# LiHaoy-ux/DQO-MAP

Measured on AMD Instinct MI355X. Metric: mapping iters/sec (fwd+bwd raster) @ 500k Gaussians 1200×680; PSNR vs ref, higher is better.
Workload: dtype f32; 1 GPU; cfg3: surfel room, ONE map of 500000 Gaussians, 1200x680, 8 object ids, SH degree 3, per-object render (object gate) + per-object masked loss (sum over objects of 0.8 L1 colour + 1.0 depth L1 on the object's own mask) + attach loss, raster fwd+bwd + Adam (6 groups); path=fused (hipGraph replays of 4 iterations each); rccl_ranks=1, backend=none (one rank), list_split=0, list_split_backward=0, graph_unroll=4, sync_mode=lazy, selfcheck=skipped, P=500000, P_visible=196562, view=room, adam=exact-sparse, adam_rows_touched=148371, attach_loss_members=49997

## Files before the change

### dqo-map_amd/csrc/dqo_capi.hip

```cpp
#include <stdarg.h>
#include <stdio.h>
#include <string.h>

#include "dqo_common.h"

static thread_local char g_err[512] = "";

void dqo_set_error(const char* fmt, ...) {
    va_list ap;
    va_start(ap, fmt);
    vsnprintf(g_err, sizeof(g_err), fmt, ap);
    va_end(ap);
}

#include <map>
#include <mutex>
#include <string>
#include <vector>
int g_dqo_profile_on = 0;
namespace {
std::mutex g_profile_mu;
struct Pending {
    std::string name;
    hipEvent_t start, stop;
// ... 65 lines not shown
                                sizeof(DqoAdamTensor), sizeof(DqoRastParamInputs), sizeof(DqoRastParamGrads), 0 ,
                                sizeof(DqoLifecycle), sizeof(DqoGrowthSample)};
    return (which >= 0 && which < (int32_t)(sizeof(sz) / sizeof(sz[0]))) ? sz[which] : 0;
}
DQO_API const char* dqo_last_error(void) { return g_err; }

DQO_API size_t dqo_rast_geom_bytes(int32_t P, int32_t W, int32_t H) {
    (void)W;
    (void)H;
    return dqo_geom_layout(nullptr, P < 0 ? 0 : P).total;
}
DQO_API size_t dqo_rast_image_bytes(int32_t W, int32_t H) { return dqo_image_layout(nullptr, W, H).total; }
DQO_API size_t dqo_rast_binning_bytes(int64_t cap) { return dqo_bin_layout(nullptr, cap < 0 ? 0 : cap, cap < 0 ? 0 : cap, 0).total; }
DQO_API size_t dqo_rast_binning_bytes_bucketed(int64_t cap, int32_t W, int32_t H, int32_t bucket) {
    if (cap < 0) cap = 0;
    if (bucket <= 0 || W <= 0 || H <= 0) return dqo_rast_binning_bytes(cap);
    return dqo_bin_layout(nullptr, cap, dqo_list_cap(cap, W, H, bucket), bucket).total;
}
DQO_API size_t dqo_rast_backward_workspace_bytes(int64_t cap) { return dqo_bwd_ws_bytes(cap); }

static int check_common(const DqoRastParams* p, const DqoRastInputs* in, const DqoRastCtx* ctx) {
    DQO_CHECK_ARG(p && in && ctx, "null params / inputs / ctx");
    DQO_CHECK_ARG(p->P >= 0 && p->W > 0 && p->H > 0, "bad sizes P=%d W=%d H=%d", p->P, p->W, p->H);
    DQO_CHECK_ARG(p->D >= 0 && p->D <= 3, "sh degree %d out of range 0..3", p->D);
    DQO_CHECK_ARG((p->W + DQO_TILE - 1) / DQO_TILE < 65536 && (p->H + DQO_TILE - 1) / DQO_TILE < 65536, "image too large");
    DQO_CHECK_ARG(in->viewmatrix && in->projmatrix && in->campos && in->bg, "viewmatrix/projmatrix/campos/bg must be given");
    if (p->P > 0) {
        DQO_CHECK_ARG(in->means3D && in->opacities, "means3D / opacities missing");
        DQO_CHECK_ARG((in->shs != nullptr) != (in->colors_precomp != nullptr),
                      "Please provide excatly one of either SHs or precomputed colors!");
        DQO_CHECK_ARG(in->cov3D_precomp == nullptr,
                      "cov3D_precomp is not supported by the depth rasteriser: its blend kernel reads scales/rotations (forward.cu:780)");
        DQO_CHECK_ARG(in->scales && in->rotations, "scales and rotations are required");
        if (in->shs) DQO_CHECK_ARG(p->M >= (p->D + 1) * (p->D + 1), "sh has %d coefficients, degree %d needs %d", p->M, p->D, (p->D + 1) * (p->D + 1));
        if (in->colors_precomp == nullptr && p->M == 0) {
            dqo_set_error("For non-RGB, provide precomputed Gaussian colors!");
            return DQO_ERR_INVALID_ARG;
        }
    }
    DQO_CHECK_ARG(ctx->geom && ctx->geom_bytes >= dqo_rast_geom_bytes(p->P, p->W, p->H), "geom buffer too small (%zu < %zu)",
                  ctx->geom_bytes, dqo_rast_geom_bytes(p->P, p->W, p->H));
    DQO_CHECK_ARG(ctx->image && ctx->image_bytes >= dqo_rast_image_bytes(p->W, p->H), "image buffer too small (%zu < %zu)",
                  ctx->image_bytes, dqo_rast_image_bytes(p->W, p->H));
    return DQO_OK;
}

// ... 221 lines not shown
```

### dqo-map_amd/csrc/dqo_common.h

```cpp
#pragma once
#include <hip/hip_runtime.h>
#include <stdint.h>

#include "../../include/dqo_raster.h"
#include "dqo_activate.h"

#define DQO_TILE 16
#define DQO_WAVE 64
#define DQO_SPREAD 64
#define DQO_GATE_OBJECTS 64
#define DQO_OBJ_SPREAD 16
#ifndef DQO_TSTRIDE
#define DQO_TSTRIDE 64
#endif

#define DQO_API __attribute__((visibility("default")))

void dqo_set_error(const char* fmt, ...);
#define DQO_CHECK_ARG(cond, ...)          \
    do {                                  \
        if (!(cond)) {                    \
            dqo_set_error(__VA_ARGS__);   \
            return DQO_ERR_INVALID_ARG;   \
        }                                 \
// ... 194 lines not shown
    }
#pragma unroll
    for (int off = 32; off > 0; off >>= 1)
#pragma unroll
        for (int c = 0; c < 4; c++) t[c] += (unsigned long long)__shfl_xor((long long)t[c], off);
    tot[0] = (double)t[0] / DQO_TAP_FIXED, tot[1] = (double)t[1], tot[2] = (double)t[2] / DQO_TAP_FIXED, tot[3] = (double)t[3];
}
__device__ __forceinline__ unsigned long long dqo_tap_fixed(float s) {
    return (s >= 0.f && s < 2147483648.f) ? (unsigned long long)((double)s * DQO_TAP_FIXED + 0.5) : ~0ull >> 1;
}
#endif

static inline int dqo_list_split(const DqoRastCtx* ctx) { return ctx->list_split <= 0 ? 0 : (ctx->list_split < 64 ? 64 : ctx->list_split); }
struct DqoImageLayout {
    uint32_t* tile_count;
    uint32_t* tile_flag;
    uint32_t* tile_cursor;
    uint2* ranges;
    uint32_t* walk4;
    uint32_t* tile_order;
    uint4* slot_info;
    float* final_T;
    uint32_t* n_contrib;
    uint32_t* hit_pos;
    uint32_t* long_tiles;
    uint32_t* split_tiles;
    size_t total;
};

static inline DqoImageLayout dqo_image_layout(void* base, int W, int H) {
    DqoImageLayout L;
    const size_t gx = (W + DQO_TILE - 1) / DQO_TILE, gy = (H + DQO_TILE - 1) / DQO_TILE;
    const size_t T = gx * gy, HW = (size_t)W * H;
    char* p = (char*)base;
    auto take = [&](size_t bytes) {
        char* r = p;
        p += dqo_align_up(bytes, 256);
        return r;
    };
    L.tile_count = (uint32_t*)take(4 * T * DQO_TSTRIDE);
    L.tile_flag = (uint32_t*)take(4 * T);
    L.tile_cursor = (uint32_t*)take(4 * T * DQO_TSTRIDE);
    L.ranges = (uint2*)take(8 * T);
    L.walk4 = (uint32_t*)take(16 * T);
    L.tile_order = (uint32_t*)take(4 * 8 * ((T + 7) / 8));
    L.slot_info = (uint4*)take(16 * 8 * ((T + 7) / 8));
    L.final_T = (float*)take(4 * HW);
    L.n_contrib = (uint32_t*)take(4 * HW);
    L.hit_pos = (uint32_t*)take(4 * HW);
    L.long_tiles = (uint32_t*)take(4 * T);
    L.split_tiles = (uint32_t*)take(4 * T);
    L.total = (size_t)(p - (char*)base);
    return L;
}

struct DqoBinLayout {
    uint4* recs;
    uint32_t* point_list;
    uint32_t* slot_list;
    uint8_t* live_q;
    uint2* slot_info;
    uint32_t* slot_gid;
    uint32_t* rec_valid;
    int64_t list_cap;
    int32_t bucket;
    size_t total;
};
static inline int64_t dqo_list_cap(int64_t cap, int W, int H, int bucket) {
    const int64_t T = (int64_t)((W + DQO_TILE - 1) / DQO_TILE) * ((H + DQO_TILE - 1) / DQO_TILE);
    return bucket > 0 ? T * bucket : cap;
}

static inline DqoBinLayout dqo_bin_layout(void* base, int64_t cap, int64_t list_cap, int bucket) {
    DqoBinLayout L;
    L.list_cap = list_cap, L.bucket = bucket;
    char* p = (char*)base;
    auto take = [&](size_t bytes) {
        char* r = p;
// ... 175 lines not shown
```

### dqo-map_amd/csrc/rast_backward_blend.hip

```cpp
#include <type_traits>

#include "dqo_common.h"
#include "dqo_cull.h"

namespace {

template <int CTRL, int ROW_MASK = 0xF>
__device__ __forceinline__ float dpp_mov(float v) {
    return __int_as_float(__builtin_amdgcn_update_dpp(0, __float_as_int(v), CTRL, ROW_MASK, 0xF, false));
}
__device__ __forceinline__ float wave_sum(float v) {
    v += dpp_mov<0xB1>(v);
    v += dpp_mov<0x4E>(v);
    v += dpp_mov<0x141>(v);
    v += dpp_mov<0x140>(v);
    v += dpp_mov<0x142, 0xA>(v);
    v += dpp_mov<0x143, 0xC>(v);
    return __int_as_float(__builtin_amdgcn_readlane(__float_as_int(v), 63));
}

__device__ __forceinline__ uint32_t row0_sum_u32(uint32_t v) {
    v += (uint32_t)__builtin_amdgcn_update_dpp(0, (int)v, 0xB1, 0xF, 0xF, false);
    v += (uint32_t)__builtin_amdgcn_update_dpp(0, (int)v, 0x4E, 0xF, 0xF, false);
    v += (uint32_t)__builtin_amdgcn_update_dpp(0, (int)v, 0x141, 0xF, 0xF, false);
// ... 165 lines not shown
        tap.loss_out[4] = r4, tap.loss_out[5] = r5, tap.loss_out[6] = r6, tap.loss_out[7] = r7;
    }
}

constexpr int BWD_THREADS = 64;
constexpr int BWD_BLK = 3 * BWD_THREADS * 4 + 3 * BWD_THREADS + 5 * BWD_THREADS;
constexpr int BWD_XCH = 5 * BWD_THREADS;

#ifndef DQO_BWD_RG
#define DQO_BWD_RG 42
#endif
constexpr int RG = DQO_BWD_RG;
constexpr int RNB = 7;
constexpr int RNV = 64;
constexpr int RLS = 8;
static_assert(RG % RNB == 0 && RG >= RNB && (RG / RNB) * RLS <= 64 && (RG / RNB) * RLS - 2 < 63, "RG: whole batches, 64 list slots per row, slot 63 free");
constexpr int R_ENT_W = 12;
constexpr int R_ENT = 0;
constexpr int R_LIST = R_ENT + (RG + 1) * R_ENT_W;
constexpr int R_NB = RG / RNB;
constexpr int R_PART = R_LIST + 4 * 64 / 2;
constexpr int R_PART_W = 4 * R_NB * RNV + 12;
constexpr int R_MPOS = R_PART + R_PART_W;
constexpr int R_MCODE = R_MPOS + 64;
constexpr int ROWS_BLK = ((R_MCODE + 16 + 3) / 4) * 4;
static_assert(R_LIST % 4 == 0 && R_PART % 4 == 0, "16-byte aligned tables");
static_assert(5 * 64 <= R_PART_W, "the depth-hit staging fits the partial table");

struct BwdTap {
    float gc, gdw;
};
__device__ __forceinline__ BwdTap tap_frame_scales(const DqoGeomLayout& g, const DqoTapDev& tap, int lane, bool report) {
    BwdTap t;
    if (!report) {
        uint32_t c1, c3;
        dqo_tap_counts(g.spread, lane, c1, c3);
        const float n_col = fmaxf((float)c1, 1.f), n_dep = fmaxf((float)c3, 1.f);
        t.gc = tap.color_weight / (3.f * n_col), t.gdw = tap.depth_weight / n_dep;
        return t;
    }
    double tot[4];
    dqo_tap_totals(g.spread, lane, tot);
    const float n_col = fmaxf((float)tot[1], 1.f), n_dep = fmaxf((float)tot[3], 1.f);
    t.gc = tap.color_weight / (3.f * n_col), t.gdw = tap.depth_weight / n_dep;
    if (report && lane == 0) {
        const float color_loss = (float)(tot[0] / (3.0 * (double)n_col)), depth_loss = (float)(tot[2] / (double)n_dep);
        tap.loss_out[0] = tap.depth_weight * depth_loss + tap.color_weight * color_loss;
        tap.loss_out[1] = color_loss, tap.loss_out[2] = depth_loss, tap.loss_out[3] = 0.f;
        tap.loss_out[4] = (float)tot[0], tap.loss_out[5] = (float)tot[1], tap.loss_out[6] = (float)tot[2], tap.loss_out[7] = (float)tot[3];
        tap.scale[0] = t.gc, tap.scale[1] = t.gdw;
// ... 8 lines not shown
                                                   const DqoTapDev& tap, const DqoGateDev& gate, const int tile, const int quad, const int wave, const int lane, uint32_t* const lds, const int skip_over,
                                                   const uint2 range) {
    constexpr bool ROWS = SEGS == 1;
    uint32_t* const blk = lds + wave * (ROWS ? ROWS_BLK : BWD_BLK);
    float4* const s_co = reinterpret_cast<float4*>(blk);
    float4* const s_xy = s_co + BWD_THREADS;
    float4* const s_rgb = s_xy + BWD_THREADS;
    int* const s_id = reinterpret_cast<int*>(s_rgb + BWD_THREADS);
    uint32_t* const s_slot = reinterpret_cast<uint32_t*>(s_id + BWD_THREADS);
    int* const s_pos = reinterpret_cast<int*>(s_slot + BWD_THREADS);
    float* const s_hit = ROWS ? reinterpret_cast<float*>(blk + R_PART) : reinterpret_cast<float*>(s_pos + BWD_THREADS);
    const int n = (int)(range.y - range.x);
    if (n == 0 || n > skip_over) return;
    const int L = min((int)img.walk4[tile * 4 + quad], n);
    if (L == 0) return;
    const int tile_x = tile % v.gx, tile_y = tile / v.gx;
    const size_t HW = (size_t)v.W * v.H;
    const uint32_t px = tile_x * DQO_TILE + (quad & 1) * 8 + dqo_lane_x(lane);
    const uint32_t py = tile_y * DQO_TILE + (quad >> 1) * 8 + dqo_lane_y(lane);
    const bool inside = px < (uint32_t)v.W && py < (uint32_t)v.H;
    const size_t pid = (size_t)v.W * py + px;
    const float pixfx = (float)px, pixfy = (float)py;
    const uint8_t* const live = bin.live_q + (size_t)quad * (size_t)bin.list_cap + range.x;
    const size_t ps = inside ? pid : (size_t)0;
    const float T_final_ld = img.final_T[ps];
    const uint32_t n_contrib_ld = img.n_contrib[ps], hit_word_ld = img.hit_pos[ps];
    int owner_ld = 0;
    if (GATE) owner_ld = gate.pobj[ps];
    float in0, in1, in2, in3, in4 = 0.f, in5 = 0.f, in6 = 0.f, in7 = 0.f;
    uint8_t mask_ld = 1;
    if (tap.scale == nullptr) {
        in0 = dL_dpixels[ps], in1 = dL_dpixels[HW + ps], in2 = dL_dpixels[2 * HW + ps], in3 = dL_ddepths[ps];
    } else {
        if (tap.mask) mask_ld = tap.mask[ps];
        in0 = tap.out_color[ps], in1 = tap.out_color[HW + ps], in2 = tap.out_color[2 * HW + ps], in3 = tap.out_depth[ps];
        in4 = tap.gt_color[ps], in5 = tap.gt_color[HW + ps], in6 = tap.gt_color[2 * HW + ps], in7 = tap.gt_depth[ps];
    }
    uint8_t lv_first = 0;
    if (ROWS) lv_first = (L - 1 - lane >= 0) ? live[L - 1 - lane] : (uint8_t)0;
    float tap_gc = 0.f, tap_gdw = 0.f;
    if (tap.scale != nullptr && !(GATE && tap.per_object)) {
        const BwdTap t = tap_frame_scales(g, tap, lane, false);
        tap_gc = t.gc, tap_gdw = t.gdw;
    }
    const float T_final = inside ? T_final_ld : 0.f;
    float T = T_final;
    const int last_contrib = inside ? (int)n_contrib_ld : 0;
    const uint32_t hit_word = inside ? hit_word_ld : 0u;
    const int hit_pos = (int)(hit_word & 0x7fffffffu);
    const bool hit_plane = (hit_word >> 31) != 0u;
    const int hit_c0 = hit_pos - 1;
    const bool has_hit = hit_pos > 0;
    const int gid_h = (int)bin.point_list[range.x + max(hit_c0, 0)];
    const uint32_t slot_h_ld = bin.slot_list[range.x + max(hit_c0, 0)];
    char* const ent_base = reinterpret_cast<char*>(blk + R_ENT);
    int* const s_mpos = reinterpret_cast<int*>(blk + R_MPOS);
    uint8_t* const s_mcode = reinterpret_cast<uint8_t*>(blk + R_MCODE);
    const int chunks = (L + BWD_THREADS - 1) / BWD_THREADS;
    int chunk_i = 0;
    unsigned long long pend = 0ull;
    uint32_t my_code = 0u;
    uint8_t lv_nx = lv_first;
    auto below = [](unsigned long long m) { return (int)__builtin_amdgcn_mbcnt_hi((uint32_t)(m >> 32), __builtin_amdgcn_mbcnt_lo((uint32_t)m, 0u)); };
    int cnt = 0;
    auto collect = [&]() -> int {
        int cnt = 0;
        while (cnt < RG) {
            if (pend == 0ull) {
                if (chunk_i >= chunks) break;
                my_code = (uint32_t)lv_nx & 0xfu;
                chunk_i++;
                const int pn = L - 1 - (chunk_i * BWD_THREADS + lane);
                lv_nx = pn >= 0 ? live[pn] : (uint8_t)0;
                pend = __builtin_amdgcn_ballot_w64(my_code != 0u);
                continue;
            }
            const int rank = below(pend);
            const bool take = ((pend >> lane) & 1ull) != 0ull && rank < RG - cnt;
            if (take) s_mpos[cnt + rank] = L - 1 - ((chunk_i - 1) * BWD_THREADS + lane), s_mcode[cnt + rank] = (uint8_t)my_code;
            const unsigned long long tm = __builtin_amdgcn_ballot_w64(take);
            cnt += (int)__popcll(tm);
            pend &= ~tm;
        }
        return cnt;
    };
    int g_id = 0;
    auto gather_ids = [&](const int c) { g_id = (int)bin.point_list[range.x + (lane < c ? s_mpos[lane] : 0)]; };
    if constexpr (ROWS) {
        cnt = collect();
        gather_ids(cnt);
    }
    int owner = (int)0x80000000;
    if (GATE) {
        if (inside) owner = owner_ld;
        if (owner < 0) owner = (int)0x80000000;
        if (tap.scale != nullptr && tap.per_object) {
            unsigned long long todo = __builtin_amdgcn_ballot_w64(owner >= 0);
            while (todo != 0ull) {
                const int f = (int)__builtin_ctzll(todo);
                const int o = __builtin_amdgcn_readlane(owner, f);
                const unsigned long long* l = g.obj_tap + ((size_t)(lane & (DQO_OBJ_SPREAD - 1)) * DQO_GATE_OBJECTS + (size_t)(o & (DQO_GATE_OBJECTS - 1))) * 4;
                static_assert(DQO_OBJ_SPREAD <= 16, "the copies sit in one DPP row");
                const uint32_t n1 = row0_sum_u32(lane < DQO_OBJ_SPREAD ? (uint32_t)l[1] : 0u);
                const uint32_t n3 = row0_sum_u32(lane < DQO_OBJ_SPREAD ? (uint32_t)l[3] : 0u);
                const float n_col = fmaxf((float)n1, 1.f), n_dep = fmaxf((float)n3, 1.f);
                const bool mine = owner == o;
                tap_gc = mine ? tap.color_weight / (3.f * n_col) : tap_gc;
                tap_gdw = mine ? tap.depth_weight / n_dep : tap_gdw;
                todo &= ~__builtin_amdgcn_ballot_w64(mine);
            }
        }
    }
    float dp0 = 0.f, dp1 = 0.f, dp2 = 0.f, ddep = 0.f;
// ... 4 lines not shown
        const bool m = mask_ld != 0 && (!(GATE && tap.per_object) || owner >= 0);
        const float d0 = in0 - in4, d1 = in1 - in5, d2 = in2 - in6;
        const float gd = in7, err = in3 - gd;
        dp0 = m ? (d0 > 0.f ? gc : (d0 < 0.f ? -gc : 0.f)) : 0.f;
        dp1 = m ? (d1 > 0.f ? gc : (d1 < 0.f ? -gc : 0.f)) : 0.f;
        dp2 = m ? (d2 > 0.f ? gc : (d2 < 0.f ? -gc : 0.f)) : 0.f;
        const bool dvalid = m && hit_pos > 0 && gd > 0.f && err < tap.add_depth_thres;
        ddep = dvalid ? (err > 0.f ? gdw : (err < 0.f ? -gdw : 0.f)) : 0.f;
    }
    if (__builtin_amdgcn_ballot_w64(dp0 != 0.f || dp1 != 0.f || dp2 != 0.f || ddep != 0.f) == 0ull) {
        if (SEGS > 1 && wave != 0) return;
        for (int p0 = 0; p0 < L; p0 += BWD_THREADS) {
            const int pos = p0 + lane;
            if (pos < L && live[pos] != 0) {
                const uint32_t slot = bin.slot_list[range.x + pos];
                if ((int64_t)slot < capacity) valid[(size_t)slot * 4 + quad] = (uint8_t)0;
            }
        }
        return;
    }
    const float bgdot = v.bg[0] * dp0 + v.bg[1] * dp1 + v.bg[2] * dp2;
    const float bg_term = -T_final * bgdot;
    const float3 ray = pixel_ray_b(px, py, v.focal_x, v.focal_y, v.cx, v.cy);
    const float4 n_np_h = g.normal_c[gid_h];
    const float4 pc_h = g.point_c[gid_h];
    float4 g_co, g_xy, g_cs;
    int g_pos = 0;
    uint32_t g_code = 0u, g_slot = 0xffffffffu;
    auto gather_records = [&](const int c) {
        const bool on = lane < c;
        g_pos = on ? s_mpos[lane] : 0;
        g_code = on ? (uint32_t)s_mcode[lane] : 0u;
        g_slot = on ? bin.slot_list[range.x + g_pos] : 0xffffffffu;
        g_co = g.conic_opacity[g_id], g_xy = g.xy_depth[g_id], g_cs = g.rgb_smax[g_id];
    };
    if constexpr (ROWS) gather_records(cnt);
    else g_co = g_xy = g_cs = make_float4(0.f, 0.f, 0.f, 0.f);
    {
        const unsigned long long hm = __builtin_amdgcn_ballot_w64(has_hit);
        if (hm != 0ull && (SEGS == 1 || wave == 0)) {
            float h[5] = {0.f, 0.f, 0.f, 0.f, 0.f};
            const uint32_t slot_h = has_hit ? slot_h_ld : 0xffffffffu;
            if (has_hit) {
#pragma clang fp contract(off)
                const float4 n_np = n_np_h, pc = pc_h;
                const float nr_f = n_np.x * ray.x + n_np.y * ray.y + n_np.z * ray.z;
                const float nr = (float)((double)nr_f + 1e-8);
                const float inv_nr = 1.0f / nr, inv_nr2 = inv_nr * inv_nr;
                const float np = n_np.x * pc.x + n_np.y * pc.y + n_np.z * pc.z;
                h[0] = hit_plane ? 0.f : ddep;
                h[1] = hit_plane ? ddep * (ray.z * inv_nr) : 0.f;
                h[2] = hit_plane ? ddep * (ray.z * (nr * pc.x - np * ray.x) * inv_nr2) : 0.f;
                h[3] = hit_plane ? ddep * (ray.z * (nr * pc.y - np * ray.y) * inv_nr2) : 0.f;
                h[4] = hit_plane ? ddep * (ray.z * (nr * pc.z - np * ray.z) * inv_nr2) : 0.f;
            }
            int leader = lane;
            unsigned long long todo = hm;
            while (todo != 0ull) {
                const int f = (int)__builtin_ctzll(todo);
                const int key = __builtin_amdgcn_readlane(hit_pos, f);
// ... 6 lines not shown
#pragma unroll
                for (int i = 0; i < 5; i++) s_hit[lane * 5 + i] = h[i];
            }
            __builtin_amdgcn_fence(__ATOMIC_RELEASE, "wavefront");
            __builtin_amdgcn_wave_barrier();
            if (has_hit && !is_leader) {
#pragma unroll
                for (int i = 0; i < 5; i++) atomicAdd(&s_hit[leader * 5 + i], h[i]);
            }
            __builtin_amdgcn_fence(__ATOMIC_ACQ_REL, "wavefront");
            __builtin_amdgcn_wave_barrier();
            if (is_leader && (int64_t)slot_h < capacity) {
                float* rec = recs + ((size_t)slot_h * 4 + quad) * 16 + 9;
#pragma unroll
                for (int i = 0; i < 5; i++) rec[i] = s_hit[lane * 5 + i];
            }
        }
    }
    if constexpr (ROWS) {
        float S0 = 0.f, S1 = 0.f, S2 = 0.f;
        uint16_t* const s_list = reinterpret_cast<uint16_t*>(blk + R_LIST);
        float* const s_part = reinterpret_cast<float*>(blk + R_PART);
        const int row = lane >> 4, sl = lane & 15;
        const char* const list_row = reinterpret_cast<const char*>(s_list) + row * 128;
        float* const part_lane = s_part + row * (R_NB * RNV) + sl * (RNV / 16);
        float* const s_zero = s_part + 4 * R_NB * RNV;
        constexpr uint32_t DUMMY = (uint32_t)(RG * R_ENT_W * 4);
        {
            if (lane < R_ENT_W) reinterpret_cast<uint32_t*>(ent_base + DUMMY)[lane] = lane == 7 ? 0xfffffffeu : 0u;
            if (lane < 12) s_zero[lane] = 0.f;
        }
        for (;;) {
            if (cnt == 0) break;
            const uint32_t code = g_code;
            if (lane < cnt) {
                const uint32_t slot_j = g_slot;
                float4* e = reinterpret_cast<float4*>(ent_base + lane * (R_ENT_W * 4));
                e[0] = make_float4(-0.5f * g_co.x, g_co.y, -0.5f * g_co.z, g_co.w);
                e[1] = make_float4(g_xy.x, g_xy.y, g_xy.w, __int_as_float(g_pos));
                e[2] = make_float4(g_cs.x, g_cs.y, g_cs.z, __uint_as_float(slot_j));
            }
            bool hit_j = false;
            {
                const int p_hi = __builtin_amdgcn_readlane(g_pos, 0), p_lo = __builtin_amdgcn_readlane(g_pos, cnt - 1);
                const bool in_grp = has_hit && hit_c0 <= p_hi && hit_c0 >= p_lo;
                unsigned long long todo = __builtin_amdgcn_ballot_w64(in_grp);
                while (todo != 0ull) {
                    const int key = __builtin_amdgcn_readlane(hit_c0, (int)__builtin_ctzll(todo));
                    hit_j = hit_j || (lane < cnt && g_pos == key);
                    todo &= ~__builtin_amdgcn_ballot_w64(in_grp && hit_c0 == key);
                }
            }
            reinterpret_cast<uint2*>(s_list)[lane] = make_uint2(DUMMY | (DUMMY << 16), DUMMY | (DUMMY << 16));
            int nsteps = 0;
            uint32_t where = 0x3f3f3f3fu;
#pragma unroll
            for (int r = 0; r < 4; r++) {
                const bool in = ((code >> r) & 1u) != 0u;
                const unsigned long long m = __builtin_amdgcn_ballot_w64(in);
                const int rk = below(m);
                const int sidx = rk + ((rk * 37) >> 8);
                if (in) s_list[r * 64 + sidx] = (uint16_t)(lane * (R_ENT_W * 4));
                where = in ? ((where & ~(0xffu << (8 * r))) | ((uint32_t)sidx << (8 * r))) : where;
                nsteps = max(nsteps, (int)__popcll(m));
            }
            const int cnt_next = collect();
            gather_ids(cnt_next);
            auto batch = [&](const int t, auto full_tag) {
                constexpr bool FULL = decltype(full_tag)::value;
                const uint4 li = *reinterpret_cast<const uint4*>(list_row + t * 16);
                const uint32_t lw[4] = {li.x, li.y, li.z, li.w};
                float v64[RNV];
#pragma unroll
                for (int i = 9 * RNB; i < RNV; i++) v64[i] = 0.f;
#pragma unroll
                for (int b = 0; b < RNB; b++) {
                    float r_c0 = 0.f, r_c1 = 0.f, r_c2 = 0.f, r_mx = 0.f, r_my = 0.f, r_ka = 0.f, r_kb = 0.f, r_kc = 0.f, r_op = 0.f;
                    if (FULL || t * RNB + b < nsteps) {
                        const uint32_t off = (b & 1) ? (lw[b >> 1] >> 16) : (lw[b >> 1] & 0xffffu);
                        const float4* e = reinterpret_cast<const float4*>(ent_base + off);
                        const float4 co = e[0], xy = e[1], cs = e[2];
                        const int c0 = __float_as_int(xy.w);
                        const float dx = xy.x - pixfx, dy = xy.y - pixfy;
                        const float power = dqo_power_pre(co.x, co.y, co.z, dx, dy);
                        const float Gx = dqo_gauss(power);
                        const float alpha_x = fminf(0.99f, co.w * Gx);
                        const bool did_color = (c0 < last_contrib) & (power <= 0.0f) & (alpha_x >= 1.0f / 255.0f) & (!GATE || __float_as_int(xy.z) == owner);
                        const float alpha = did_color ? alpha_x : 0.f;
                        const float G = did_color ? Gx : 0.f;
                        const float inv_1ma = dqo_rcp(1.f - alpha);
// ... 11 lines not shown
                        r_c1 = dchannel_dcolor * dp1;
                        r_c2 = dchannel_dcolor * dp2;
                        r_mx = qx, r_my = qy;
                        r_ka = qx * dx;
                        r_kb = qx * dy;
                        r_kc = qy * dy;
                        r_op = q;
                    }
                    v64[9 * b + 0] = r_c0, v64[9 * b + 1] = r_c1, v64[9 * b + 2] = r_c2, v64[9 * b + 3] = r_mx, v64[9 * b + 4] = r_my;
                    v64[9 * b + 5] = r_ka, v64[9 * b + 6] = r_kb, v64[9 * b + 7] = r_kc, v64[9 * b + 8] = r_op;
                }
                float out[4];
                row_reduce64(v64, out, lane);
                *reinterpret_cast<float4*>(part_lane + t * RNV) = make_float4(out[0], out[1], out[2], out[3]);
            };
            {
                int t = 0;
                for (; (t + 1) * RNB <= nsteps; t++) batch(t, std::true_type{});
                if (t * RNB < nsteps) batch(t, std::false_type{});
            }
            const uint32_t slot_j = lane < cnt ? reinterpret_cast<const uint32_t*>(ent_base)[lane * R_ENT_W + 11] : 0xffffffffu;
            if (lane < cnt && (int64_t)slot_j < capacity) {
                const float* pr[4];
#pragma unroll
                for (int r = 0; r < 4; r++) {
                    const uint32_t sidx = (where >> (8 * r)) & 0xffu;
                    pr[r] = sidx == 63u ? s_zero : s_part + (r * R_NB + (int)(sidx / RLS)) * RNV + (int)(sidx % RLS) * 9;
                }
                float acc[9];
#pragma unroll
                for (int f = 0; f < 9; f++) acc[f] = ((pr[0][f] + pr[1][f]) + pr[2][f]) + pr[3][f];
                float* rec = recs + ((size_t)slot_j * 4 + quad) * 16;
                reinterpret_cast<float4*>(rec)[0] = make_float4(acc[0], acc[1], acc[2], acc[3]);
                reinterpret_cast<float4*>(rec)[1] = make_float4(acc[4], acc[5], acc[6], acc[7]);
                rec[8] = acc[8];
                valid[(size_t)slot_j * 4 + quad] = hit_j ? (uint8_t)3 : (uint8_t)1;
            }
            cnt = cnt_next;
            if (cnt == 0) break;
            gather_records(cnt);
        }
        return;
    }
    float S0 = 0.f, S1 = 0.f, S2 = 0.f;
    const int lane_b = lane / 9, lane_f = lane - 9 * lane_b;
    cnt = 0;
    auto batch = [&](const int k0, auto full_tag) {
        constexpr bool FULL = decltype(full_tag)::value;
        float v64[64];
#pragma unroll
        for (int i = 9 * BWD_NB; i < 64; i++) v64[i] = 0.f;
        uint32_t hitmask = 0u;
#pragma unroll
        for (int b = 0; b < BWD_NB; b++) {
            const int k = k0 + b;
            float r_c0 = 0.f, r_c1 = 0.f, r_c2 = 0.f, r_mx = 0.f, r_my = 0.f, r_ka = 0.f, r_kb = 0.f, r_kc = 0.f, r_op = 0.f;
            if (FULL || k < cnt) {
                const float4 co = s_co[k], xy = s_xy[k], cs = s_rgb[k];
                const int c0 = s_pos[k];
// ... 20 lines not shown
                r_c2 = dchannel_dcolor * dp2;
                r_mx = qx, r_my = qy;
                r_ka = qx * dx;
                r_kb = qx * dy;
                r_kc = qy * dy;
                r_op = q;

                if (__builtin_amdgcn_ballot_w64(hit_c0 == c0) != 0ull) hitmask |= 1u << b;
            }
            v64[9 * b + 0] = r_c0, v64[9 * b + 1] = r_c1, v64[9 * b + 2] = r_c2, v64[9 * b + 3] = r_mx, v64[9 * b + 4] = r_my;
            v64[9 * b + 5] = r_ka, v64[9 * b + 6] = r_kb, v64[9 * b + 7] = r_kc, v64[9 * b + 8] = r_op;
        }
        const float tot = wave_reduce64(v64, lane);
        const int kb = k0 + lane_b;
        if (lane < 9 * BWD_NB && (FULL || kb < cnt)) {
            const uint32_t slot = s_slot[kb];
            if ((int64_t)slot < capacity) recs[((size_t)slot * 4 + quad) * 16 + lane_f] = tot;
        }
        if (lane < BWD_NB && (FULL || k0 + lane < cnt)) {
            const uint32_t slot = s_slot[k0 + lane];
            if ((int64_t)slot < capacity) valid[(size_t)slot * 4 + quad] = ((hitmask >> lane) & 1u) ? (uint8_t)3 : (uint8_t)1;
        }
    };
    auto gather = [&](int pos, bool is_live) {
        const unsigned long long lm = __builtin_amdgcn_ballot_w64(is_live);
        cnt = (int)__popcll(lm);
        const int myk = (int)__popcll(lm & ((1ull << lane) - 1ull));
        if (is_live) {
            const int id = (int)bin.point_list[range.x + pos];
            s_id[myk] = id;
            s_pos[myk] = pos;
            s_slot[myk] = bin.slot_list[range.x + pos];
            const float4 co_g = g.conic_opacity[id];
            s_co[myk] = make_float4(-0.5f * co_g.x, co_g.y, -0.5f * co_g.z, co_g.w);
            s_xy[myk] = g.xy_depth[id];
            s_rgb[myk] = g.rgb_smax[id];
        }
    };
    auto walk_chunk = [&]() {
        int k0 = 0;
        for (; k0 + BWD_NB <= cnt; k0 += BWD_NB) batch(k0, std::true_type{});
        if (k0 < cnt) batch(k0, std::false_type{});
    };
    float* const s_x = reinterpret_cast<float*>(lds + SEGS * BWD_BLK);
    float T_round = T_final, R0 = 0.f, R1 = 0.f, R2 = 0.f;
    int p_nx = L - 1 - (wave * BWD_THREADS + lane);
    lv_nx = p_nx >= 0 ? live[p_nx] : (uint8_t)0;
    for (int r = 0; r * SEGS < chunks; r++) {
        const int pos = L - 1 - ((r * SEGS + wave) * BWD_THREADS + lane);
        const bool is_live = lv_nx != 0;
        {
            const int pn = pos - SEGS * BWD_THREADS;
            lv_nx = pn >= 0 ? live[pn] : (uint8_t)0;
        }
        gather(pos, is_live);
        float Q = 1.f, B = 1.f, A0 = 0.f, A1 = 0.f, A2 = 0.f;
#pragma unroll 2
        for (int k = 0; k < cnt; k++) {
            const float4 co = s_co[k], xy = s_xy[k], cs = s_rgb[k];
            const int c0 = s_pos[k];
            const float dx = xy.x - pixfx, dy = xy.y - pixfy;
            const float power = dqo_power_pre(co.x, co.y, co.z, dx, dy);
            const float alpha_x = fminf(0.99f, co.w * dqo_gauss(power));
            const bool did_color = c0 < last_contrib && power <= 0.0f && alpha_x >= 1.0f / 255.0f && (!GATE || __float_as_int(xy.w) == owner);
            const float alpha = did_color ? alpha_x : 0.f;
            Q *= dqo_rcp(1.f - alpha);
            A0 += alpha * (cs.x - A0), A1 += alpha * (cs.y - A1), A2 += alpha * (cs.z - A2);
            B *= 1.f - alpha;
        }
        float* const xw = s_x + ((r & 1) * SEGS + wave) * BWD_XCH + lane;
        xw[0 * BWD_THREADS] = Q, xw[1 * BWD_THREADS] = B, xw[2 * BWD_THREADS] = A0, xw[3 * BWD_THREADS] = A1, xw[4 * BWD_THREADS] = A2;
        __syncthreads();
        float Tn = T_round, N0 = R0, N1 = R1, N2 = R2;
#pragma unroll
        for (int j = 0; j < SEGS; j++) {
            if (j == wave) T = Tn, S0 = N0, S1 = N1, S2 = N2;
            const float* xj = s_x + ((r & 1) * SEGS + j) * BWD_XCH + lane;
            const float Bj = xj[1 * BWD_THREADS];
// ... 89 lines not shown
    }
    double tot[4];
    dqo_tap_totals(g.spread, (int)threadIdx.x, tot);
    if (threadIdx.x != 0) return;
    const float n_col = fmaxf((float)tot[1], 1.f), n_dep = fmaxf((float)tot[3], 1.f);
    const float color_loss = (float)(tot[0] / (3.0 * (double)n_col)), depth_loss = (float)(tot[2] / (double)n_dep);
    tap.loss_out[0] = tap.depth_weight * depth_loss + tap.color_weight * color_loss;
    tap.loss_out[1] = color_loss, tap.loss_out[2] = depth_loss, tap.loss_out[3] = 0.f;
    tap.loss_out[4] = (float)tot[0], tap.loss_out[5] = (float)tot[1], tap.loss_out[6] = (float)tot[2], tap.loss_out[7] = (float)tot[3];
    tap.scale[0] = tap.color_weight / (3.f * n_col), tap.scale[1] = tap.depth_weight / n_dep;
}

}

int dqo_launch_tap_report(const DqoGeomLayout& g, const DqoTapDev& tap, hipStream_t s) {
    DQO_LAUNCH("tap_report_kernel", tap_report_kernel, dim3(1), dim3(64), s, g, tap);
    return DQO_OK;
}

int dqo_launch_blend_backward(const DqoView& v, const DqoGeomLayout& g, const DqoImageLayout& img, const DqoBinLayout& bin, int T,
                              const float* dL_dcolor, const float* dL_ddepth, DqoGradRec* recs, uint8_t* valid, int64_t capacity,
                              const DqoTapDev& tap, const DqoGateDev& gate, int list_split, hipStream_t s) {
    float* r = reinterpret_cast<float*>(recs);
    if (list_split > 0) {
        const dim3 grid(2 * BSPLIT_GRID + 8 * (((T + 7) / 8 + 1) / 2)), block(BWD_THREADS * BSPLIT_RUNS);
        static const hipError_t raised = [] {
            const int bytes = BSPLIT_LDS_WORDS * 4;
            hipError_t e = hipFuncSetAttribute(reinterpret_cast<const void*>(&blend_backward_split_kernel<true>),
                                               hipFuncAttributeMaxDynamicSharedMemorySize, bytes);
            if (e == hipSuccess)
                e = hipFuncSetAttribute(reinterpret_cast<const void*>(&blend_backward_split_kernel<false>),
                                        hipFuncAttributeMaxDynamicSharedMemorySize, bytes);
            return e;
        }();
        if (raised != hipSuccess) {
            dqo_set_error("hipFuncSetAttribute(blend_backward_split_kernel, MaxDynamicSharedMemorySize) failed: %s", hipGetErrorString(raised));
            return DQO_ERR_LAUNCH;
        }
        if (gate.gobj != nullptr)
            DQO_LAUNCH_SMEM("blend_backward_kernel", blend_backward_split_kernel<true>, grid, block, (size_t)BSPLIT_LDS_WORDS * 4, s, v, g, img, bin,
                            dL_dcolor, dL_ddepth, r, valid, capacity, tap, gate);
        else
            DQO_LAUNCH_SMEM("blend_backward_kernel", blend_backward_split_kernel<false>, grid, block, (size_t)BSPLIT_LDS_WORDS * 4, s, v, g, img, bin,
                            dL_dcolor, dL_ddepth, r, valid, capacity, tap, gate);
        return DQO_OK;
    }
// ... 10 lines not shown
```

### dqo-map_amd/csrc/rast_forward_blend.hip

```cpp
#include "dqo_common.h"
#include "dqo_cull.h"

namespace {

__device__ __forceinline__ float3 pixel_ray(uint32_t px, uint32_t py, float fx, float fy, float cx, float cy) {
#pragma clang fp contract(off)
    float rx = ((float)px - cx) / fx, ry = ((float)py - cy) / fy, rz = 1.0f;
    const float n = 1.0f / sqrtf(rx * rx + ry * ry + rz * rz);
    return make_float3(rx * n, ry * n, rz * n);
}

struct HitEval {
    float t, den, hit_z;
};
__device__ __forceinline__ HitEval eval_hit(const float3 ray, const float4 n_np) {
#pragma clang fp contract(off)
    HitEval h;
    h.den = ray.x * n_np.x + ray.y * n_np.y + ray.z * n_np.z;
    h.t = (float)((double)n_np.w / ((double)h.den + 1e-8));
    h.hit_z = h.t * ray.z;
    return h;
}

constexpr int FWD_THREADS = 64;
// ... 161 lines not shown
        while (todo != 0ull) {
            const int o = __builtin_amdgcn_readlane(owner, (int)__builtin_ctzll(todo));
            present |= 1ull << (o & 63);
            todo &= ~__builtin_amdgcn_ballot_w64(owner == o);
        }
        mixed = __popcll(present) > 1;
    }

    if (n == 0) {
        const bool rendered = img.tile_flag[tile] != 0u;
        if (SEGS > 1 && wave != 0) return;
        if (inside) {
            out.out_color[pix_id] = rendered ? v.bg[0] : 0.f;
            out.out_color[HW + pix_id] = rendered ? v.bg[1] : 0.f;
            out.out_color[2 * HW + pix_id] = rendered ? v.bg[2] : 0.f;
            out.out_depth[pix_id] = 0.f;
            out.out_hit_depth[pix_id] = rendered ? -1 : 0;
            out.out_hit_color[pix_id] = rendered ? -1 : 0;
            out.out_hit_color_weight[pix_id] = 0.f;
            out.out_hit_depth_weight[pix_id] = 0.f;
            out.out_T[pix_id] = 1.f;
            img.final_T[pix_id] = 1.f;
            img.n_contrib[pix_id] = 0;
            img.hit_pos[pix_id] = 0;
        }
        if (lane == 0) img.walk4[tile * 4 + quad] = 0;
        if (tap.scale != nullptr)
            loss_tap_wave(tap, g, inside, pix_id, HW, rendered ? v.bg[0] : 0.f, rendered ? v.bg[1] : 0.f, rendered ? v.bg[2] : 0.f, 0.f,
                          rendered ? -1 : 0, lane, owner);
        return;
    }

    const float qx0 = (float)(tile_x * DQO_TILE + (quad & 1) * 8), qy0 = (float)(tile_y * DQO_TILE + (quad >> 1) * 8);
    const float pixfx = (float)px, pixfy = (float)py;
    const float static_gate = (inside && (!GATE || owner >= 0)) ? 1.f : 0.f;
    lanemask alive_m = __builtin_amdgcn_ballot_w64(static_gate != 0.f);
    lanemask fixed_m = 0ull;
    const float hit_thr = fmaxf(v.opaque_thr, 1.0f / 255.0f);
    const float thr255 = 1.0f / 255.0f, T_thr = v.T_thr;
    float T = 1.0f, end_T = 1.0f;
    uint32_t last_contributor = 0, hit_pos = 0;
    float C0 = 0.f, C1 = 0.f, C2 = 0.f;
    float depth_ = 0.f;
    int hit_id = -1, hit_color_id = -1;
    float color_weight_max = -1.f, hit_depth_weight = 0.f;
    uint8_t* live = bin.live_q + (size_t)quad * (size_t)bin.list_cap + range.x;

// ... 186 lines not shown
            const int la = __float_as_int(q[12 * FWD_THREADS]);
            if (la > last_alive) last_alive = la, T = q[11 * FWD_THREADS];
        }
    }
    if (__builtin_amdgcn_ballot_w64(hit_id != -1) != 0ull) {
        const int hid = max(hit_id, 0);
        const float4 n_np = g.normal_c[hid];
        const float raw_smax = g.point_c[hid].w;
        const float hit_zc = g.xy_depth[hid].z, hit_smax = g.rgb_smax[hid].w;
        if (hit_id != -1) {
            const float3 ray = pixel_ray(px, py, v.focal_x, v.focal_y, v.cx, v.cy);
            const HitEval h = eval_hit(ray, n_np);
            const float angle_distance = fabsf(h.den);
            const float depth_distance = fabsf(h.hit_z - hit_zc);
            depth_ = (depth_distance <= hit_smax * v.depth_thr && angle_distance >= v.normal_thr) ? h.hit_z : hit_zc;
            const bool plane_b = depth_distance <= v.depth_thr * raw_smax && angle_distance >= v.normal_thr;
            hit_pos |= plane_b ? 0x80000000u : 0u;
        }
    }
    const float oc0 = C0 + T * v.bg[0], oc1 = C1 + T * v.bg[1], oc2 = C2 + T * v.bg[2];
    if (inside) {
        img.final_T[pix_id] = end_T;
        img.n_contrib[pix_id] = last_contributor;
        img.hit_pos[pix_id] = hit_pos;
        out.out_color[pix_id] = oc0;
        out.out_color[HW + pix_id] = oc1;
        out.out_color[2 * HW + pix_id] = oc2;
        out.out_depth[pix_id] = depth_;
        out.out_hit_depth[pix_id] = hit_id;
        out.out_hit_color[pix_id] = hit_color_id;
        out.out_hit_color_weight[pix_id] = fmaxf(color_weight_max, 0.f);
        out.out_hit_depth_weight[pix_id] = hit_depth_weight;
        out.out_T[pix_id] = end_T;
    }
    int w = inside ? (int)max(last_contributor, hit_pos & 0x7fffffffu) : 0;
    w = (int)dqo_wave_max_u32((uint32_t)w, lane);
    if (lane == 0) img.walk4[tile * 4 + quad] = (uint32_t)w;
    if (tap.scale != nullptr) loss_tap_wave(tap, g, inside, pix_id, HW, oc0, oc1, oc2, depth_, hit_id, lane, owner);
}

#ifndef FWD_WPB
#define FWD_WPB 1
#endif
#ifndef FWD_PF
#define FWD_PF false
#endif
#ifndef FWD_MINW
// ... 79 lines not shown
```

Before: 2416 iter/s.

## Pack Gaussian ids with live codes in backward blend and store hit id in forward

The backward blend kernel now reads the Gaussian id from point_list together with the live code during list collection. It packs both into one 28+4-bit word staged in LDS, so the separate dependent id gather before the record gather goes away. The forward pass also stores the hit Gaussian id next to hit_pos, which removes an indirect point_list lookup in backward. The hit/where bookkeeping moves into LDS tables and the hit-membership test becomes a ballot mask. In exchange there are extra coalesced id loads per chunk, a larger hit_pos buffer, more LDS per block, and a new limit of P < 2^28.

Result: no change. 2403 iter/s (-0.6%).

```diff
diff --git a/dqo-map_amd/csrc/dqo_capi.hip b/dqo-map_amd/csrc/dqo_capi.hip
--- a/dqo-map_amd/csrc/dqo_capi.hip
+++ b/dqo-map_amd/csrc/dqo_capi.hip
@@ -111,6 +111,7 @@
 static int check_common(const DqoRastParams* p, const DqoRastInputs* in, const DqoRastCtx* ctx) {
     DQO_CHECK_ARG(p && in && ctx, "null params / inputs / ctx");
     DQO_CHECK_ARG(p->P >= 0 && p->W > 0 && p->H > 0, "bad sizes P=%d W=%d H=%d", p->P, p->W, p->H);
+    DQO_CHECK_LIVE_ID(p->P);
     DQO_CHECK_ARG(p->D >= 0 && p->D <= 3, "sh degree %d out of range 0..3", p->D);
     DQO_CHECK_ARG((p->W + DQO_TILE - 1) / DQO_TILE < 65536 && (p->H + DQO_TILE - 1) / DQO_TILE < 65536, "image too large");
     DQO_CHECK_ARG(in->viewmatrix && in->projmatrix && in->campos && in->bg, "viewmatrix/projmatrix/campos/bg must be given");
diff --git a/dqo-map_amd/csrc/dqo_common.h b/dqo-map_amd/csrc/dqo_common.h
--- a/dqo-map_amd/csrc/dqo_common.h
+++ b/dqo-map_amd/csrc/dqo_common.h
@@ -240,7 +240,7 @@
     uint4* slot_info;
     float* final_T;
     uint32_t* n_contrib;
-    uint32_t* hit_pos;
+    uint2* hit_pos;
     uint32_t* long_tiles;
     uint32_t* split_tiles;
     size_t total;
@@ -265,13 +265,15 @@
     L.slot_info = (uint4*)take(16 * 8 * ((T + 7) / 8));
     L.final_T = (float*)take(4 * HW);
     L.n_contrib = (uint32_t*)take(4 * HW);
-    L.hit_pos = (uint32_t*)take(4 * HW);
+    L.hit_pos = (uint2*)take(8 * HW);
     L.long_tiles = (uint32_t*)take(4 * T);
     L.split_tiles = (uint32_t*)take(4 * T);
     L.total = (size_t)(p - (char*)base);
     return L;
 }
 
+#define DQO_LIVE_ID_LIMIT (1 << 28)
+#define DQO_CHECK_LIVE_ID(P) DQO_CHECK_ARG((P) < DQO_LIVE_ID_LIMIT, "P = %d: the backward blend packs a Gaussian index into 28 bits, P must stay below 2^28", (int)(P))
 struct DqoBinLayout {
     uint4* recs;
     uint32_t* point_list;
diff --git a/dqo-map_amd/csrc/rast_backward_blend.hip b/dqo-map_amd/csrc/rast_backward_blend.hip
--- a/dqo-map_amd/csrc/rast_backward_blend.hip
+++ b/dqo-map_amd/csrc/rast_backward_blend.hip
@@ -211,10 +211,14 @@
 constexpr int R_PART = R_LIST + 4 * 64 / 2;
 constexpr int R_PART_W = 4 * R_NB * RNV + 12;
 constexpr int R_MPOS = R_PART + R_PART_W;
-constexpr int R_MCODE = R_MPOS + 64;
-constexpr int ROWS_BLK = ((R_MCODE + 16 + 3) / 4) * 4;
+constexpr int R_MWORD = R_MPOS + 64;
+constexpr int R_WHERE = R_MWORD + 64;
+constexpr int R_HITC = R_WHERE + 64;
+constexpr int R_CHUNK = R_HITC + 64;
+constexpr int ROWS_BLK = ((R_CHUNK + 64 + 3) / 4) * 4;
 static_assert(R_LIST % 4 == 0 && R_PART % 4 == 0, "16-byte aligned tables");
 static_assert(5 * 64 <= R_PART_W, "the depth-hit staging fits the partial table");
+static_assert(ROWS_BLK * 4 * 16 <= 160 * 1024, "four waves per SIMD fit the CU's LDS");
 
 struct BwdTap {
     float gc, gdw;
@@ -269,9 +273,11 @@
     const size_t pid = (size_t)v.W * py + px;
     const float pixfx = (float)px, pixfy = (float)py;
     const uint8_t* const live = bin.live_q + (size_t)quad * (size_t)bin.list_cap + range.x;
+    const uint32_t* const ids = bin.point_list + range.x;
     const size_t ps = inside ? pid : (size_t)0;
     const float T_final_ld = img.final_T[ps];
-    const uint32_t n_contrib_ld = img.n_contrib[ps], hit_word_ld = img.hit_pos[ps];
+    const uint32_t n_contrib_ld = img.n_contrib[ps];
+    const uint2 hit_ld = img.hit_pos[ps];
     int owner_ld = 0;
     if (GATE) owner_ld = gate.pobj[ps];
     float in0, in1, in2, in3, in4 = 0.f, in5 = 0.f, in6 = 0.f, in7 = 0.f;
@@ -283,8 +289,8 @@
         in0 = tap.out_color[ps], in1 = tap.out_color[HW + ps], in2 = tap.out_color[2 * HW + ps], in3 = tap.out_depth[ps];
         in4 = tap.gt_color[ps], in5 = tap.gt_color[HW + ps], in6 = tap.gt_color[2 * HW + ps], in7 = tap.gt_depth[ps];
     }
-    uint8_t lv_first = 0;
-    if (ROWS) lv_first = (L - 1 - lane >= 0) ? live[L - 1 - lane] : (uint8_t)0;
+    uint32_t lv_first = 0u, id_first = 0u;
+    if (ROWS && L - 1 - lane >= 0) lv_first = live[L - 1 - lane], id_first = ids[L - 1 - lane];
     float tap_gc = 0.f, tap_gdw = 0.f;
     if (tap.scale != nullptr && !(GATE && tap.per_object)) {
         const BwdTap t = tap_frame_scales(g, tap, lane, false);
@@ -293,21 +299,23 @@
     const float T_final = inside ? T_final_ld : 0.f;
     float T = T_final;
     const int last_contrib = inside ? (int)n_contrib_ld : 0;
-    const uint32_t hit_word = inside ? hit_word_ld : 0u;
+    const uint32_t hit_word = inside ? hit_ld.x : 0u;
     const int hit_pos = (int)(hit_word & 0x7fffffffu);
     const bool hit_plane = (hit_word >> 31) != 0u;
     const int hit_c0 = hit_pos - 1;
     const bool has_hit = hit_pos > 0;
-    const int gid_h = (int)bin.point_list[range.x + max(hit_c0, 0)];
+    const int gid_h = has_hit ? (int)hit_ld.y : 0;
     const uint32_t slot_h_ld = bin.slot_list[range.x + max(hit_c0, 0)];
+    const float4 n_np_h = g.normal_c[gid_h];
+    const float4 pc_h = g.point_c[gid_h];
     char* const ent_base = reinterpret_cast<char*>(blk + R_ENT);
     int* const s_mpos = reinterpret_cast<int*>(blk + R_MPOS);
-    uint8_t* const s_mcode = reinterpret_cast<uint8_t*>(blk + R_MCODE);
+    uint32_t* const s_mword = reinterpret_cast<uint32_t*>(blk + R_MWORD);
     const int chunks = (L + BWD_THREADS - 1) / BWD_THREADS;
     int chunk_i = 0;
     unsigned long long pend = 0ull;
-    uint32_t my_code = 0u;
-    uint8_t lv_nx = lv_first;
+    uint32_t* const s_chunk = reinterpret_cast<uint32_t*>(blk + R_CHUNK);
+    uint32_t lv_nx = lv_first, id_nx = id_first;
     auto below = [](unsigned long long m) { return (int)__builtin_amdgcn_mbcnt_hi((uint32_t)(m >> 32), __builtin_amdgcn_mbcnt_lo((uint32_t)m, 0u)); };
     int cnt = 0;
     auto collect = [&]() -> int {
@@ -315,27 +323,41 @@
         while (cnt < RG) {
             if (pend == 0ull) {
                 if (chunk_i >= chunks) break;
-                my_code = (uint32_t)lv_nx & 0xfu;
+                const uint32_t my_word = (id_nx << 4) | (lv_nx & 0xfu);
+                s_chunk[lane] = my_word;
                 chunk_i++;
                 const int pn = L - 1 - (chunk_i * BWD_THREADS + lane);
-                lv_nx = pn >= 0 ? live[pn] : (uint8_t)0;
-                pend = __builtin_amdgcn_ballot_w64(my_code != 0u);
+                lv_nx = 0u;
+                if (pn >= 0) lv_nx = live[pn], id_nx = ids[pn];
+                pend = __builtin_amdgcn_ballot_w64((my_word & 0xfu) != 0u);
                 continue;
             }
             const int rank = below(pend);
             const bool take = ((pend >> lane) & 1ull) != 0ull && rank < RG - cnt;
-            if (take) s_mpos[cnt + rank] = L - 1 - ((chunk_i - 1) * BWD_THREADS + lane), s_mcode[cnt + rank] = (uint8_t)my_code;
+            if (take) s_mpos[cnt + rank] = L - 1 - ((chunk_i - 1) * BWD_THREADS + lane), s_mword[cnt + rank] = s_chunk[lane];
             const unsigned long long tm = __builtin_amdgcn_ballot_w64(take);
             cnt += (int)__popcll(tm);
             pend &= ~tm;
         }
         return cnt;
     };
-    int g_id = 0;
-    auto gather_ids = [&](const int c) { g_id = (int)bin.point_list[range.x + (lane < c ? s_mpos[lane] : 0)]; };
+    float4 g_co, g_xy, g_cs;
+    int g_pos = 0;
+    uint32_t g_code = 0u, g_slot = 0xffffffffu;
+    auto gather_records = [&](const int c) {
+        const bool on = lane < c;
+        const uint32_t w = on ? s_mword[lane] : 0u;
+        const int g_id = (int)(w >> 4);
+        g_pos = on ? s_mpos[lane] : 0;
+        g_code = w & 0xfu;
+        g_slot = on ? bin.slot_list[range.x + g_pos] : 0xffffffffu;
+        g_co = g.conic_opacity[g_id], g_xy = g.xy_depth[g_id], g_cs = g.rgb_smax[g_id];
+    };
     if constexpr (ROWS) {
         cnt = collect();
-        gather_ids(cnt);
+        gather_records(cnt);
+    } else {
+        g_co = g_xy = g_cs = make_float4(0.f, 0.f, 0.f, 0.f);
     }
     int owner = (int)0x80000000;
     if (GATE) {
@@ -386,20 +408,6 @@
     const float bgdot = v.bg[0] * dp0 + v.bg[1] * dp1 + v.bg[2] * dp2;
     const float bg_term = -T_final * bgdot;
     const float3 ray = pixel_ray_b(px, py, v.focal_x, v.focal_y, v.cx, v.cy);
-    const float4 n_np_h = g.normal_c[gid_h];
-    const float4 pc_h = g.point_c[gid_h];
-    float4 g_co, g_xy, g_cs;
-    int g_pos = 0;
-    uint32_t g_code = 0u, g_slot = 0xffffffffu;
-    auto gather_records = [&](const int c) {
-        const bool on = lane < c;
-        g_pos = on ? s_mpos[lane] : 0;
-        g_code = on ? (uint32_t)s_mcode[lane] : 0u;
-        g_slot = on ? bin.slot_list[range.x + g_pos] : 0xffffffffu;
-        g_co = g.conic_opacity[g_id], g_xy = g.xy_depth[g_id], g_cs = g.rgb_smax[g_id];
-    };
-    if constexpr (ROWS) gather_records(cnt);
-    else g_co = g_xy = g_cs = make_float4(0.f, 0.f, 0.f, 0.f);
     {
         const unsigned long long hm = __builtin_amdgcn_ballot_w64(has_hit);
         if (hm != 0ull && (SEGS == 1 || wave == 0)) {
@@ -452,6 +460,7 @@
         uint16_t* const s_list = reinterpret_cast<uint16_t*>(blk + R_LIST);
         float* const s_part = reinterpret_cast<float*>(blk + R_PART);
         const int row = lane >> 4, sl = lane & 15;
+        reinterpret_cast<int*>(blk + R_HITC)[lane] = hit_c0;
         const char* const list_row = reinterpret_cast<const char*>(s_list) + row * 128;
         float* const part_lane = s_part + row * (R_NB * RNV) + sl * (RNV / 16);
         float* const s_zero = s_part + 4 * R_NB * RNV;
@@ -470,15 +479,16 @@
                 e[1] = make_float4(g_xy.x, g_xy.y, g_xy.w, __int_as_float(g_pos));
                 e[2] = make_float4(g_cs.x, g_cs.y, g_cs.z, __uint_as_float(slot_j));
             }
-            bool hit_j = false;
+            unsigned long long hit_jm = 0ull;
             {
                 const int p_hi = __builtin_amdgcn_readlane(g_pos, 0), p_lo = __builtin_amdgcn_readlane(g_pos, cnt - 1);
-                const bool in_grp = has_hit && hit_c0 <= p_hi && hit_c0 >= p_lo;
+                const int hc = reinterpret_cast<const int*>(blk + R_HITC)[lane];
+                const bool in_grp = hc >= 0 && hc <= p_hi && hc >= p_lo;
                 unsigned long long todo = __builtin_amdgcn_ballot_w64(in_grp);
                 while (todo != 0ull) {
-                    const int key = __builtin_amdgcn_readlane(hit_c0, (int)__builtin_ctzll(todo));
-                    hit_j = hit_j || (lane < cnt && g_pos == key);
-                    todo &= ~__builtin_amdgcn_ballot_w64(in_grp && hit_c0 == key);
+                    const int key = __builtin_amdgcn_readlane(hc, (int)__builtin_ctzll(todo));
+                    hit_jm |= __builtin_amdgcn_ballot_w64(lane < cnt && g_pos == key);
+                    todo &= ~__builtin_amdgcn_ballot_w64(in_grp && hc == key);
                 }
             }
             reinterpret_cast<uint2*>(s_list)[lane] = make_uint2(DUMMY | (DUMMY << 16), DUMMY | (DUMMY << 16));
@@ -495,7 +505,7 @@
                 nsteps = max(nsteps, (int)__popcll(m));
             }
             const int cnt_next = collect();
-            gather_ids(cnt_next);
+            reinterpret_cast<uint32_t*>(blk + R_WHERE)[lane] = where;
             auto batch = [&](const int t, auto full_tag) {
                 constexpr bool FULL = decltype(full_tag)::value;
                 const uint4 li = *reinterpret_cast<const uint4*>(list_row + t * 16);
@@ -553,9 +563,10 @@
             const uint32_t slot_j = lane < cnt ? reinterpret_cast<const uint32_t*>(ent_base)[lane * R_ENT_W + 11] : 0xffffffffu;
             if (lane < cnt && (int64_t)slot_j < capacity) {
                 const float* pr[4];
+                const uint32_t where_j = reinterpret_cast<const uint32_t*>(blk + R_WHERE)[lane];
 #pragma unroll
                 for (int r = 0; r < 4; r++) {
-                    const uint32_t sidx = (where >> (8 * r)) & 0xffu;
+                    const uint32_t sidx = (where_j >> (8 * r)) & 0xffu;
                     pr[r] = sidx == 63u ? s_zero : s_part + (r * R_NB + (int)(sidx / RLS)) * RNV + (int)(sidx % RLS) * 9;
                 }
                 float acc[9];
@@ -565,7 +576,7 @@
                 reinterpret_cast<float4*>(rec)[0] = make_float4(acc[0], acc[1], acc[2], acc[3]);
                 reinterpret_cast<float4*>(rec)[1] = make_float4(acc[4], acc[5], acc[6], acc[7]);
                 rec[8] = acc[8];
-                valid[(size_t)slot_j * 4 + quad] = hit_j ? (uint8_t)3 : (uint8_t)1;
+                valid[(size_t)slot_j * 4 + quad] = ((hit_jm >> lane) & 1ull) != 0ull ? (uint8_t)3 : (uint8_t)1;
             }
             cnt = cnt_next;
             if (cnt == 0) break;
@@ -632,12 +643,13 @@
             if ((int64_t)slot < capacity) valid[(size_t)slot * 4 + quad] = ((hitmask >> lane) & 1u) ? (uint8_t)3 : (uint8_t)1;
         }
     };
-    auto gather = [&](int pos, bool is_live) {
+    auto gather = [&](int pos, uint32_t word) {
+        const bool is_live = (word & 0xfu) != 0u;
         const unsigned long long lm = __builtin_amdgcn_ballot_w64(is_live);
         cnt = (int)__popcll(lm);
         const int myk = (int)__popcll(lm & ((1ull << lane) - 1ull));
         if (is_live) {
-            const int id = (int)bin.point_list[range.x + pos];
+            const int id = (int)(word >> 4);
             s_id[myk] = id;
             s_pos[myk] = pos;
             s_slot[myk] = bin.slot_list[range.x + pos];
@@ -655,15 +667,17 @@
     float* const s_x = reinterpret_cast<float*>(lds + SEGS * BWD_BLK);
     float T_round = T_final, R0 = 0.f, R1 = 0.f, R2 = 0.f;
     int p_nx = L - 1 - (wave * BWD_THREADS + lane);
-    lv_nx = p_nx >= 0 ? live[p_nx] : (uint8_t)0;
+    lv_nx = 0u;
+    if (p_nx >= 0) lv_nx = live[p_nx], id_nx = ids[p_nx];
     for (int r = 0; r * SEGS < chunks; r++) {
         const int pos = L - 1 - ((r * SEGS + wave) * BWD_THREADS + lane);
-        const bool is_live = lv_nx != 0;
+        const uint32_t word = (id_nx << 4) | (lv_nx & 0xfu);
         {
             const int pn = pos - SEGS * BWD_THREADS;
-            lv_nx = pn >= 0 ? live[pn] : (uint8_t)0;
-        }
-        gather(pos, is_live);
+            lv_nx = 0u;
+            if (pn >= 0) lv_nx = live[pn], id_nx = ids[pn];
+        }
+        gather(pos, word);
         float Q = 1.f, B = 1.f, A0 = 0.f, A1 = 0.f, A2 = 0.f;
 #pragma unroll 2
         for (int k = 0; k < cnt; k++) {
@@ -799,6 +813,7 @@
                               const float* dL_dcolor, const float* dL_ddepth, DqoGradRec* recs, uint8_t* valid, int64_t capacity,
                               const DqoTapDev& tap, const DqoGateDev& gate, int list_split, hipStream_t s) {
     float* r = reinterpret_cast<float*>(recs);
+    DQO_CHECK_LIVE_ID(v.P);
     if (list_split > 0) {
         const dim3 grid(2 * BSPLIT_GRID + 8 * (((T + 7) / 8 + 1) / 2)), block(BWD_THREADS * BSPLIT_RUNS);
         static const hipError_t raised = [] {
diff --git a/dqo-map_amd/csrc/rast_forward_blend.hip b/dqo-map_amd/csrc/rast_forward_blend.hip
--- a/dqo-map_amd/csrc/rast_forward_blend.hip
+++ b/dqo-map_amd/csrc/rast_forward_blend.hip
@@ -207,7 +207,7 @@
             out.out_T[pix_id] = 1.f;
             img.final_T[pix_id] = 1.f;
             img.n_contrib[pix_id] = 0;
-            img.hit_pos[pix_id] = 0;
+            img.hit_pos[pix_id] = make_uint2(0u, 0u);
         }
         if (lane == 0) img.walk4[tile * 4 + quad] = 0;
         if (tap.scale != nullptr)
@@ -440,7 +440,7 @@
     if (inside) {
         img.final_T[pix_id] = end_T;
         img.n_contrib[pix_id] = last_contributor;
-        img.hit_pos[pix_id] = hit_pos;
+        img.hit_pos[pix_id] = make_uint2(hit_pos, (uint32_t)max(hit_id, 0));
         out.out_color[pix_id] = oc0;
         out.out_color[HW + pix_id] = oc1;
         out.out_color[2 * HW + pix_id] = oc2;
```
